# guzba/zippy

Measured on NVIDIA H100. Metric: compress_level1_gzip_input_throughput, higher is better.
Workload: dtype u8

## Files before the change

zippy_b200/csrc/zb_deflate.cu:

```cuda
#include "zb_device.cuh"
#include "zb_kernels.h"
#include "zb_huff_warp.cuh"

#define LZ_THREADS (ZB_WARPS_PER_CHUNK * 32)
#define LZ_HASH_BITS 11
#define LZ_TABLE_ENTRIES (1 << LZ_HASH_BITS)
#define LZ_PRESEED 2048
#ifndef ZB_LZ1_RESOLVE_WINNER
#define ZB_LZ1_RESOLVE_WINNER 0
#endif
#define LZ_LANE_CAP 32

#define LZ_PIECE_BYTES ZB_REC_PIECE_BYTES
#define LZ_PHASES (ZB_SUB_BYTES / LZ_PIECE_BYTES)
#define LZ_PHASE_BYTES (ZB_CHUNK_BYTES / LZ_PHASES)
#define LZ_PHASE_HIST 1024
#define LZ_BATCH_LPW 2
#define LZ_BATCH_WINDOWS (32 / LZ_BATCH_LPW)
static_assert(LZ_PIECE_BYTES * ZB_WARPS_PER_CHUNK == LZ_PHASE_BYTES, "one piece per warp and phase");
static_assert(LZ_PIECE_BYTES / ZB_WINDOW % LZ_BATCH_WINDOWS == 0, "a batch of windows never straddles two pieces");

#define LZ_SM_DATA 0
#define LZ_SM_DATA_BYTES (LZ_PHASE_BYTES + LZ_PHASE_HIST + 64 + 384)
#define LZ_SM_TABLE (LZ_SM_DATA + LZ_SM_DATA_BYTES)
#define LZ_SM_TABLE_BYTES (ZB_WARPS_PER_CHUNK * LZ_TABLE_ENTRIES * 2)
#define LZ_SM_HIST (LZ_SM_TABLE + LZ_SM_TABLE_BYTES)
#define LZ_SM_HIST_BYTES (ZB_WARPS_PER_CHUNK * ZB_HIST_WORDS * 4)
#define LZ_SM_RING (LZ_SM_HIST + LZ_SM_HIST_BYTES)
#define LZ_SM_RING_BYTES (ZB_WARPS_PER_CHUNK * LZ_BATCH_WINDOWS * ZB_MATCH_SLOTS * 4)
#define LZ_SM_LMUL (LZ_SM_RING + LZ_SM_RING_BYTES)
#define LZ_LMUL_PIECE 33
#define LZ_LMUL_PQ 49
#define LZ_SM_LMUL_BYTES (56 * 4)
#define LZ_SM_PART (LZ_SM_LMUL + LZ_SM_LMUL_BYTES)
#define LZ_SM_PART_BYTES (ZB_WARPS_PER_CHUNK * 24)
#define LZ_SM_BAR (LZ_SM_PART + LZ_SM_PART_BYTES)
#define LZ_SM_TOTAL (LZ_SM_BAR + 16)
static_assert(LZ_TABLE_ENTRIES * 2 >= 4096, "a warp's table region must hold the CRC step table");
static_assert(3 * (LZ_SM_TOTAL + 1024) <= 233472, "three CTAs per SM");
static_assert(LZ_SM_PART % 8 == 0 && LZ_SM_TABLE % 16 == 0, "alignment");

__device__ __forceinline__ uint32_t lz_hash(uint32_t v) { return (v * 0x9E3779B1u) >> (32 - LZ_HASH_BITS); }
__device__ __forceinline__ uint32_t shl_clamp(uint32_t x, uint32_t n) {
  uint32_t r;
  asm("shl.b32 %0, %1, %2;" : "=r"(r) : "r"(x), "r"(n));
  return r;
}
__device__ __forceinline__ uint32_t low_mask(uint32_t n) { return shl_clamp(1u, n) - 1u; }

__device__ __forceinline__ uint32_t lz_final_rec(uint32_t mlen, uint32_t dist, int &lc, int &dc) {
  uint32_t le, de;
  lc = (int)zb_len_code_bf(mlen, le);
  dc = (int)zb_dist_code_bf(dist, de);
  return (uint32_t)lc | (le << 5) | ((uint32_t)dc << 10) | (de << 15);
}


__device__ __forceinline__ void lz_select(const uint8_t *data, uint32_t off0, uint32_t wb, uint32_t b1, uint32_t cur,
                                          uint32_t nvalid, uint32_t &m, uint32_t dist, uint32_t *ring_slot,
                                          uint32_t &sel, uint32_t &ism, uint32_t &endw) {
  const int lane = zb_lane();
  const uint32_t mm = __ballot_sync(ZB_FULL, m != 0);
  endw = 0;
  ism = 0;
  if (mm) {
    const uint32_t lbit = 1u << lane;
    const uint32_t endp = (uint32_t)lane + m;
    const uint32_t rest = shl_clamp(1u, endp) ? (mm >> endp) : 0u;
    uint32_t nc = rest ? endp + (uint32_t)(__ffs((int)rest) - 1) : 32u;
    uint32_t vis = 1u << (cur + (uint32_t)(__ffs((int)(mm >> cur)) - 1));
#pragma unroll
    for (int r = 0; r < 3; r++) {
      vis |= __reduce_or_sync(ZB_FULL, (vis & lbit) ? shl_clamp(1u, nc) : 0u);
      const uint32_t t = __shfl_sync(ZB_FULL, nc, (int)(nc & 31u));
      nc = nc < 32u ? t : 32u;
    }
    ism = vis;
    const int lastm = 31 - __clz((int)ism);
    const uint32_t cov = (ism & lbit) ? (low_mask(endp) & ~low_mask((uint32_t)lane)) : 0u;
    const uint32_t covered = __reduce_or_sync(ZB_FULL, cov);
    uint32_t mlast = __shfl_sync(ZB_FULL, m, lastm);
    if (mlast >= LZ_LANE_CAP) {
      const uint32_t md = __shfl_sync(ZB_FULL, dist, lastm);
      const uint32_t pos = wb + (uint32_t)lastm;
      const uint32_t off = off0 + pos + LZ_LANE_CAP + 8u * (uint32_t)lane;
      uint32_t x0 = zb_ld32_unaligned(data, off) ^ zb_ld32_unaligned(data, off - md);
      uint32_t x1 = zb_ld32_unaligned(data, off + 4) ^ zb_ld32_unaligned(data, off + 4 - md);
      uint32_t nm = x0 ? ((uint32_t)(__ffs((int)x0) - 1) >> 3) : 4u + (x1 ? ((uint32_t)(__ffs((int)x1) - 1) >> 3) : 4u);
      uint32_t stop = __ballot_sync(ZB_FULL, nm < 8u);
      if (stop) {
        int first = __ffs((int)stop) - 1;
        mlast = LZ_LANE_CAP + 8u * (uint32_t)first + __shfl_sync(ZB_FULL, nm, first);
      } else {
        mlast = LZ_LANE_CAP + 256u;
      }
      mlast = min(mlast, min((uint32_t)ZB_MAX_MATCH, b1 - pos));
      if (lane == lastm) m = mlast;
    }
    sel = ism | (~covered & ~low_mask(cur) & low_mask(nvalid));
    endw = (uint32_t)lastm + mlast;
    if (ism & lbit) {
      uint32_t rank = (uint32_t)__popc(ism & (lbit - 1u));
      ring_slot[rank] = (m - 3u) | ((dist - 1u) << 9);
    }
  } else {
    sel = low_mask(nvalid) & ~low_mask(cur);
  }
}

template <int LPW, bool LITS>
__device__ __forceinline__ void lz_batch_pass(const uint8_t *wdata, bool active, uint32_t ksel, uint32_t kism,
                                              const uint32_t *ring_win, uint32_t *whist, uint2 *gmask_w,
                                              uint32_t *grecs_piece, uint32_t &rec_base) {
  constexpr int NW = 32 / LPW;
  const uint32_t part = (uint32_t)zb_lane() / NW, wi = (uint32_t)zb_lane() % NW;
  if (active && part == 0) *gmask_w = make_uint2(ksel, kism);
  const uint32_t im = active ? kism : 0u;
  const uint32_t pm = (0xffffffffu >> (32 - 32 / LPW)) << (part * (32 / LPW));
  uint32_t s = (LITS && active) ? (ksel & ~kism & pm) : 0u;
  while (s) {
    const uint32_t bit = (uint32_t)(__ffs((int)s) - 1);
    s &= s - 1;
    const uint32_t sy = wdata[bit];
    atomicAdd(&whist[sy >> 1], 1u << ((sy & 1u) * 16u));
  }
  const uint32_t nmatch = (uint32_t)__popc(im);
  uint32_t incl = nmatch;
#pragma unroll
  for (int o = 1; o < NW; o <<= 1) {
    const uint32_t t = __shfl_up_sync(ZB_FULL, incl, o, NW);
    if (wi >= (uint32_t)o) incl += t;
  }
  uint32_t *grecs_w = grecs_piece + rec_base + incl - nmatch;
  rec_base += __shfl_sync(ZB_FULL, incl, NW - 1);
  for (uint32_t k = part; k < nmatch; k += LPW) {
    const uint32_t raw = ring_win[k];
    int lc, dc;
    const uint32_t fin = lz_final_rec((raw & 511u) + 3u, (raw >> 9) + 1u, lc, dc);
    grecs_w[k] = fin;
    const uint32_t s1 = 257u + (uint32_t)lc, s2 = (uint32_t)ZB_NUM_LITLEN + (uint32_t)dc;
    atomicAdd(&whist[s1 >> 1], 1u << ((s1 & 1u) * 16u));
    atomicAdd(&whist[s2 >> 1], 1u << ((s2 & 1u) * 16u));
  }
}

#ifndef ZB_LZ1_STAGE_CLOCKS
#define ZB_LZ1_STAGE_CLOCKS 0
#endif
enum { LZS_WAIT, LZS_CHECKSUM, LZS_SEED, LZS_PROBE, LZS_EXTEND, LZS_SELECT, LZS_BATCH, LZS_BARRIER, LZS_N };
#if ZB_LZ1_STAGE_CLOCKS
__device__ unsigned long long zb_lz1_stage_clk[LZS_N];
#define LZ_CLK_DECL                          \
  unsigned long long clk_acc[LZS_N] = {};    \
  long long clk_t = clock64();
#define LZ_CLK(s)                            \
  if (MODE == 1) {                           \
    const long long clk_n = clock64();       \
    clk_acc[s] += (unsigned long long)(clk_n - clk_t); \
    clk_t = clk_n;                           \
  }
#define LZ_CLK_PUBLISH()                                                                           \
  if (MODE == 1 && lane == 0) {                                                                    \
    _Pragma("unroll") for (int s_ = 0; s_ < LZS_N; s_++) atomicAdd(&zb_lz1_stage_clk[s_], clk_acc[s_]); \
  }
extern "C" int zb200_lz1_stage_clocks(unsigned long long *out) {
  unsigned long long zero[LZS_N] = {};
  if (cudaMemcpyFromSymbol(out, zb_lz1_stage_clk, sizeof(zero)) != cudaSuccess) return -1;
  return cudaMemcpyToSymbol(zb_lz1_stage_clk, zero, sizeof(zero)) == cudaSuccess ? 0 : -1;
}
#else
#define LZ_CLK_DECL
#define LZ_CLK(s)
#define LZ_CLK_PUBLISH()
#endif

template <int MODE, int CK>
__global__ void __launch_bounds__(LZ_THREADS, 3)
    k_lz(const uint8_t *__restrict__ src, const ZbChunkDesc *__restrict__ desc, uint2 *__restrict__ masks,
         uint32_t *__restrict__ recs, uint16_t *__restrict__ hist, ZbChunkCheck *__restrict__ chk,
         const ZbCrcTables *__restrict__ tabs, uint32_t max_dist) {
  extern __shared__ __align__(128) uint8_t smem[];
  uint8_t *data = smem + LZ_SM_DATA;
  uint16_t *table_all = reinterpret_cast<uint16_t *>(smem + LZ_SM_TABLE);
  uint32_t *hist_all = reinterpret_cast<uint32_t *>(smem + LZ_SM_HIST);
  uint32_t *ring_all = reinterpret_cast<uint32_t *>(smem + LZ_SM_RING);
  uint32_t *lane_mul = reinterpret_cast<uint32_t *>(smem + LZ_SM_LMUL);
  uint64_t *part = reinterpret_cast<uint64_t *>(smem + LZ_SM_PART);
  uint64_t *bar = reinterpret_cast<uint64_t *>(smem + LZ_SM_BAR);

  const uint32_t chunk = blockIdx.x;
  const ZbChunkDesc d = desc[chunk];
  const uint32_t len = d.len;
  const int tid = (int)threadIdx.x, lane = tid & 31;
  const int warp = (int)__reduce_max_sync(ZB_FULL, (uint32_t)tid >> 5);

  if (tid == 0) {
    zb_mbar_init(bar, 1);
    zb_fence_mbar_init();
  }
  __syncthreads();
  const uint32_t mis = (uint32_t)((uintptr_t)(src + d.src_off) & 15u);

  uint16_t *table = table_all + warp * LZ_TABLE_ENTRIES;
  uint32_t *ring = ring_all + warp * LZ_BATCH_WINDOWS * ZB_MATCH_SLOTS;
  uint2 *gmask = masks + (size_t)chunk * ZB_WINDOWS_PER_CHUNK;
  uint32_t acc_crc = 0;
  uint64_t acc_a = 0, acc_b = 0;
  LZ_CLK_DECL

  for (uint32_t ph = 0; ph < LZ_PHASES; ph++) {
    const uint32_t pbase = ph * LZ_PHASE_BYTES;
    if (ph && pbase >= len) break;
    const uint32_t sbase = ph ? pbase - LZ_PHASE_HIST : 0u;
    if (ph) __syncthreads();
    LZ_CLK(LZS_BARRIER)
    if (tid == 0 && len) {
      zb_fence_proxy_async();
      zb_stage_chunk(data, src + d.src_off + sbase, min(len, pbase + LZ_PHASE_BYTES + 384u) - sbase, bar);
    }
    if (CK & ZB_CK_CRC) {
      uint32_t *crc_tab = reinterpret_cast<uint32_t *>(table);
      for (int i = lane; i < 1024; i += 32) crc_tab[i] = (&tabs->mul1024[0][0])[i];
    }
    if (ph == 0) {
      for (int i = tid; i < ZB_WARPS_PER_CHUNK * ZB_HIST_WORDS; i += LZ_THREADS) hist_all[i] = 0;
      if (tid < 33) lane_mul[tid] = tabs->lane_mul[tid];
      if (tid >= 64 && tid < 80) lane_mul[LZ_LMUL_PIECE + tid - 64] = tabs->piece_mul[tid - 64];
      if (tid >= 96 && tid < 100) lane_mul[LZ_LMUL_PQ + tid - 96] = tabs->pq_mul[tid - 96];
      __syncthreads();
    } else {
      __syncwarp();
    }
    if (len) zb_mbar_wait(bar, ph & 1u);
    LZ_CLK(LZS_WAIT)

    const uint32_t b0 = pbase + (uint32_t)warp * LZ_PIECE_BYTES;
    if (b0 >= len) continue;
    const uint32_t b1 = min(b0 + LZ_PIECE_BYTES, len);
    const uint32_t doff = mis - sbase;
    uint32_t *whist = hist_all + (b0 / ZB_SUB_BYTES) * ZB_HIST_WORDS;

    if (CK) {
      ZbCheck c = zb_warp_checksums<LZ_PIECE_BYTES, LZ_LMUL_PQ, CK>(data, doff + b0, b1 - b0,
                                                                    reinterpret_cast<const uint32_t *>(table), lane_mul);
      const uint32_t after = len - b1;
      if (after) {
        if (CK & ZB_CK_CRC) {
          const uint32_t shift = ((after & (LZ_PIECE_BYTES - 1)) == 0) ? lane_mul[LZ_LMUL_PIECE + after / LZ_PIECE_BYTES]
                                                                       : zb_xpow8_t(tabs->pow2, after);
          c.crc_raw = zb_gf2_mul(c.crc_raw, shift);
        }
        if (CK & ZB_CK_ADLER) c.b_sum += (uint64_t)after * c.a_sum;
      }
      acc_crc ^= c.crc_raw;
      acc_a += c.a_sum;
      acc_b += c.b_sum;
      __syncwarp();
    }
    LZ_CLK(LZS_CHECKSUM)

    if (MODE == 1) {
      uint4 ff = make_uint4(~0u, ~0u, ~0u, ~0u);
      uint4 *t4 = reinterpret_cast<uint4 *>(table);
      for (int i = lane; i < LZ_TABLE_ENTRIES * 2 / 16; i += 32) t4[i] = ff;
      __syncwarp();
      for (uint32_t s = b0 - min((uint32_t)LZ_PRESEED, b0 - sbase); s < b0; s += 32) {
        const uint32_t p = s + (uint32_t)lane;
        const bool can = p + 4 <= len;
        const uint32_t h = lz_hash(zb_ld32_unaligned(data, doff + p));
        if (can) table[h] = (uint16_t)p;
#if ZB_LZ1_RESOLVE_WINNER
        __syncwarp();
        for (;;) {
          const bool lost = can && table[h] < (uint16_t)p;
          if (!__any_sync(ZB_FULL, lost)) break;
          if (lost) table[h] = (uint16_t)p;
          __syncwarp();
        }
#endif
      }
      __syncwarp();
    }
    LZ_CLK(LZS_SEED)
    uint32_t entry = b0;
    uint32_t ksel = 0, kism = 0;
    uint32_t *grecs = recs + (size_t)chunk * ZB_RECS_PER_CHUNK + (b0 >> 2);
    uint32_t rec_base = 0;
    const uint32_t bl = (uint32_t)lane & (LZ_BATCH_WINDOWS - 1u);
    for (uint32_t wb = b0; wb < b1; wb += 32) {
      const uint32_t win = wb >> 5, slot = win & (LZ_BATCH_WINDOWS - 1u);
      uint32_t sel = 0, ism = 0;
      if (entry < wb + 32) {
        const uint32_t p = wb + (uint32_t)lane;
        const uint32_t nvalid = min(32u, b1 - wb);
        const uint32_t cur = entry - wb;
        uint32_t m = 0, c = 0, lit = 0;
        if (MODE == 2) {
          const uint32_t x = doff + p;
          lit = data[x];
          const uint32_t eq0 = __ballot_sync(ZB_FULL, p != 0u && lit == data[x - 1u]);
          const uint32_t eq1 = __ballot_sync(ZB_FULL, data[x + 32u] == data[x + 31u]);
          const uint32_t ahead = __funnelshift_r(eq0, eq1, (uint32_t)lane);
          const uint32_t run = ahead == ~0u ? (uint32_t)LZ_LANE_CAP : (uint32_t)(__ffs((int)~ahead) - 1);
          const uint32_t limit = p < b1 ? b1 - p : 0u;
          const uint32_t r = run < (uint32_t)LZ_LANE_CAP ? min(run, limit) : run;
          if (p >= entry && r >= 3u && limit >= 3u) m = r;
          c = p - 1u;
        }
        if (MODE == 1) {
          const uint32_t *wp = reinterpret_cast<const uint32_t *>(data) + ((doff + p) >> 2);
          const uint32_t sp = ((doff + p) & 3u) * 8u;
          const uint32_t p0 = wp[0], p1 = wp[1];
          const uint32_t v = __funnelshift_r(p0, p1, sp);
          lit = v & 255u;
          const bool can = (p + 4 <= len);
          const uint32_t h = lz_hash(v);
          c = table[h];
          __syncwarp();
          if (can) table[h] = (uint16_t)p;
#if ZB_LZ1_RESOLVE_WINNER
          __syncwarp();
          for (;;) {
            const bool lost = can && table[h] < (uint16_t)p;
            if (!__any_sync(ZB_FULL, lost)) break;
            if (lost) table[h] = (uint16_t)p;
            __syncwarp();
          }
#endif
          LZ_CLK(LZS_PROBE)
          const uint32_t limit = p < b1 ? min((uint32_t)ZB_MAX_MATCH, b1 - p) : 0u;
          if (can && c < p && p - c <= max_dist && p >= entry && limit >= ZB_MIN_MATCH) {
            const uint32_t *wc = reinterpret_cast<const uint32_t *>(data) + ((doff + c) >> 2);
            const uint32_t sc = ((doff + c) & 3u) * 8u;
            uint32_t hp = p1, hc = wc[1];
            uint32_t np = wp[2], nq = wc[2], np2 = wp[3], nq2 = wc[3];
            if (__funnelshift_r(wc[0], hc, sc) == v) {
              m = 4;
#pragma unroll 1
              for (int k = 2;; k += 2) {
                const uint32_t x = __funnelshift_r(hp, np, sp) ^ __funnelshift_r(hc, nq, sc);
                const uint32_t x2 = __funnelshift_r(np, np2, sp) ^ __funnelshift_r(nq, nq2, sc);
                if (x) {
                  m += (uint32_t)(__ffs((int)x) - 1) >> 3;
                  break;
                }
                if (k == LZ_LANE_CAP / 4) {
                  m += 4;
                  break;
                }
                if (x2) {
                  m += 4u + ((uint32_t)(__ffs((int)x2) - 1) >> 3);
                  break;
                }
                m += 8;
                hp = np2;
                hc = nq2;
                np = wp[k + 2];
                nq = wc[k + 2];
                np2 = wp[k + 3];
                nq2 = wc[k + 3];
              }
              if (m < LZ_LANE_CAP) m = min(m, limit);
            }
          }
          LZ_CLK(LZS_EXTEND)
        }
        uint32_t endw;
        lz_select(data, doff, wb, b1, cur, nvalid, m, p - c, ring + slot * ZB_MATCH_SLOTS, sel, ism, endw);
        entry = wb + max(endw, nvalid);
        if (MODE != 0 && ((sel & ~ism) >> lane & 1u)) atomicAdd(&whist[lit >> 1], 1u << ((lit & 1u) * 16u));
        LZ_CLK(LZS_SELECT)
      }
      if (bl == slot) {
        ksel = sel;
        kism = ism;
      }
      if (slot == LZ_BATCH_WINDOWS - 1u || wb + 32 >= b1) {
        __syncwarp();
        const uint32_t bwin = win - slot + bl;
        lz_batch_pass<LZ_BATCH_LPW, MODE == 0>(data + (uint32_t)(doff + (bwin << 5)), bl <= slot, ksel, kism, ring + bl * ZB_MATCH_SLOTS,
                                    whist, gmask + bwin, grecs, rec_base);
        ksel = kism = 0;
        __syncwarp();
      }
      LZ_CLK(LZS_BATCH)
    }
  }
  if (lane == 0) {
    part[warp * 3 + 0] = acc_crc;
    part[warp * 3 + 1] = acc_a;
    part[warp * 3 + 2] = acc_b;
  }
  __syncthreads();
  {
    uint32_t *gh = reinterpret_cast<uint32_t *>(hist + (size_t)chunk * ZB_WARPS_PER_CHUNK * ZB_HIST_SYMS);
    for (int i = tid; i < ZB_WARPS_PER_CHUNK * ZB_HIST_WORDS; i += LZ_THREADS) gh[i] = hist_all[i];
  }
  LZ_CLK(LZS_BARRIER)
  LZ_CLK_PUBLISH()
  if (tid == 0) {
    uint32_t raw = 0;
    uint64_t a = 0, b = 0;
    for (int w = 0; w < ZB_WARPS_PER_CHUNK; w++) {
      raw ^= (uint32_t)part[w * 3 + 0];
      a += part[w * 3 + 1];
      b += part[w * 3 + 2];
    }
    ZbChunkCheck cc;
    cc.crc_raw = raw;
    cc.adler = (CK & ZB_CK_ADLER) ? zb_adler_from_sums(a % ZB_ADLER_MOD, b % ZB_ADLER_MOD, len) : 0u;
    chk[chunk] = cc;
  }
}

#define LZ2_HIST 32768
#define LZ2_SEG_BYTES ZB_SUB_BYTES
#define LZ2_SEGS ((ZB_CHUNK_BYTES + LZ2_HIST) / LZ2_SEG_BYTES)
#define LZ2_BUCKET_BITS 11
#define LZ2_BUCKETS (1 << LZ2_BUCKET_BITS)
#define LZ2_TABLES_PER_CTA (ZB_WARPS_PER_CHUNK + LZ2_SEGS)
#define LZ2_RING_WINDOWS 8
#define LZ2_SM_DATA_BYTES (ZB_CHUNK_BYTES + LZ2_HIST + 64 + 384)
#define LZ2_SM_HIST (LZ2_SM_DATA_BYTES)
#define LZ2_SM_RING (LZ2_SM_HIST + LZ_SM_HIST_BYTES)
#define LZ2_SM_RING_BYTES (ZB_WARPS_PER_CHUNK * LZ2_RING_WINDOWS * ZB_MATCH_SLOTS * 4)
#define LZ2_SM_CRC (LZ2_SM_RING + LZ2_SM_RING_BYTES)
#define LZ2_SM_LMUL (LZ2_SM_CRC + 4096)
#define LZ2_SM_PART (LZ2_SM_LMUL + LZ_SM_LMUL_BYTES)
#define LZ2_SM_LIST (LZ2_SM_PART + LZ_SM_PART_BYTES)
#define LZ2_SM_BAR (LZ2_SM_LIST + 8 * LZ_THREADS * 2)
#define LZ2_SM_TOTAL (LZ2_SM_BAR + 16)
static_assert(2 * (LZ2_SM_TOTAL + 1024) <= 233472, "two CTAs per SM");

#ifndef LZ2_CTAS_PER_SM
#define LZ2_CTAS_PER_SM 1
#endif
#ifndef LZ2_STATIC_BITS
#define LZ2_STATIC_BITS 13
#endif
__device__ __forceinline__ uint32_t lz2_hash_mul(uint32_t v) { return v * 0x9E3779B1u; }
__device__ __forceinline__ uint32_t lz2_hash(uint32_t v) { return lz2_hash_mul(v) >> (32 - LZ2_BUCKET_BITS); }

__device__ __forceinline__ uint2 lz2_push(uint2 b, uint32_t e) {
  uint2 r;
  r.y = __funnelshift_l(b.x, b.y, 16);
  r.x = (b.x << 16) | (e & 0xffffu);
  return r;
}

__device__ __forceinline__ void lz2_clear_table(uint2 *tab, int bytes = LZ2_BUCKETS * 8) {
  const uint4 ff = make_uint4(~0u, ~0u, ~0u, ~0u);
  uint4 *t4 = reinterpret_cast<uint4 *>(tab);
  for (int i = zb_lane(); i < bytes / 16; i += 32) __stcg(&t4[i], ff);
}

__device__ __forceinline__ uint2 lz2_probe_insert(uint2 *tab, uint32_t h, bool can, uint32_t qwin, uint32_t &grp) {
  const int lane = zb_lane();
  grp = __match_any_sync(ZB_FULL, can ? h : (0x80000000u | (uint32_t)lane));
  uint2 old = make_uint2(~0u, ~0u);
  if (can) old = __ldcg(&tab[h]);
  __syncwarp();
  if (can && lane == 31 - __clz((int)grp)) {
    uint2 nb = old;
    for (uint32_t g = grp; g; g &= g - 1) nb = lz2_push(nb, qwin + (uint32_t)(__ffs((int)g) - 1));
    __stcg(&tab[h], nb);
  }
  __syncwarp();
  return old;
}

struct Lz2Pos {
  const uint32_t *data32;
  uint32_t poff;
  uint32_t q;
  uint32_t v;
  uint32_t lim;
  uint32_t limit, stop;
};

#define LZ2_LIST 8
__device__ __forceinline__ void lz2_verify(const Lz2Pos &P, uint32_t e, bool search, uint16_t *dl, uint32_t &n) {
  const uint32_t d = (P.q - e) & 0xffffu;
  if (!search || (d - 1u) >= P.lim) return;
  const uint32_t co = P.poff - d;
  const uint32_t *wc = P.data32 + (co >> 2);
  if (__funnelshift_r(wc[0], wc[1], (co & 3u) * 8u) != P.v) return;
  if (n < LZ2_LIST) dl[n * (uint32_t)LZ_THREADS] = (uint16_t)d;
  n += n < LZ2_LIST ? 1u : 0u;
}
__device__ __forceinline__ void lz2_extend(const Lz2Pos &P, const uint8_t *data, uint32_t d, uint32_t good, uint32_t &m,
                                           uint32_t &dist, int &budget) {
  const uint32_t co = P.poff - d;
  budget--;
  if (m >= 4 && data[co + m] != data[P.poff + m]) {
    if (m >= good && budget > 1) budget = 1;
    return;
  }
  const uint32_t *wc = P.data32 + (co >> 2);
  const uint32_t sc = (co & 3u) * 8u;
  const uint32_t *wp = P.data32 + (P.poff >> 2);
  const uint32_t sp = (P.poff & 3u) * 8u;
  uint32_t hp = wp[1], hc = wc[1];
  uint32_t mc = 4;
#pragma unroll 1
  for (int j = 2; j <= LZ_LANE_CAP / 4; j++) {
    const uint32_t np = wp[j], nq = wc[j];
    const uint32_t x = __funnelshift_r(hp, np, sp) ^ __funnelshift_r(hc, nq, sc);
    if (x) {
      mc += (uint32_t)(__ffs((int)x) - 1) >> 3;
      break;
    }
    mc += 4;
    hp = np;
    hc = nq;
  }
  mc = min(mc, P.limit);
  if (mc > m) {
    m = mc;
    dist = d;
  }
  if (m >= good && budget > 1) budget = 1;
}

__device__ __forceinline__ void stage_dict_chunk(uint8_t *data, const uint8_t *chunk, uint32_t len, uint32_t hb,
                                                 const uint8_t *wend, uint64_t *bar) {
  const uint32_t cmis = (uint32_t)((uintptr_t)chunk & 15u);
  const uint32_t mis = (cmis - hb) & 15u, a0 = hb + mis - cmis;
  const uint32_t cbytes = (cmis + len + 15u) & ~15u;
  zb_mbar_expect_tx(bar, a0 + cbytes);
  for (uint32_t done = 0; done < a0;) {
    const uint32_t n = min(a0 - done, 32768u);
    zb_tma_load_1d(data + done, wend - hb - mis + done, n, bar);
    done += n;
  }
  for (uint32_t done = 0; done < cbytes;) {
    const uint32_t n = min(cbytes - done, 32768u);
    zb_tma_load_1d(data + a0 + done, chunk - cmis + done, n, bar);
    done += n;
  }
}
__device__ __forceinline__ void fix_dict_head(uint8_t *data, const uint8_t *chunk, uint32_t hb, const uint8_t *wend) {
  const uint32_t cmis = (uint32_t)((uintptr_t)chunk & 15u);
  const uint32_t mis = (cmis - hb) & 15u;
  const uint32_t q = hb - min(hb, cmis) + threadIdx.x;
  if (q < hb) {
    data[mis + q] = wend[(int)q - (int)hb];
    zb_fence_proxy_async();
  }
}

template <bool DICT, int MINM = ZB_MIN_MATCH>
__global__ void __launch_bounds__(LZ_THREADS, 2)
    k_lz2(const uint8_t *__restrict__ src, const ZbChunkDesc *__restrict__ desc, uint2 *__restrict__ masks,
          uint32_t *__restrict__ recs, uint16_t *__restrict__ hist, ZbChunkCheck *__restrict__ chk,
          const ZbCrcTables *__restrict__ tabs, uint2 *__restrict__ tables, uint32_t n_chunks, ZbLz2Params prm,
          const ZbMemberDict *__restrict__ mdict) {
  extern __shared__ __align__(128) uint8_t smem[];
  uint8_t *data = smem;
  uint32_t *hist_all = reinterpret_cast<uint32_t *>(smem + LZ2_SM_HIST);
  uint32_t *ring_all = reinterpret_cast<uint32_t *>(smem + LZ2_SM_RING);
  uint32_t *crc_tab = reinterpret_cast<uint32_t *>(smem + LZ2_SM_CRC);
  uint32_t *lane_mul = reinterpret_cast<uint32_t *>(smem + LZ2_SM_LMUL);
  uint64_t *part = reinterpret_cast<uint64_t *>(smem + LZ2_SM_PART);
  uint64_t *bar = reinterpret_cast<uint64_t *>(smem + LZ2_SM_BAR);
  const int tid = (int)threadIdx.x, lane = tid & 31, warp = tid >> 5;
  uint16_t *dlist = reinterpret_cast<uint16_t *>(smem + LZ2_SM_LIST) + tid;
  uint32_t *whist = hist_all + warp * ZB_HIST_WORDS;
  uint32_t *ring = ring_all + warp * LZ2_RING_WINDOWS * ZB_MATCH_SLOTS;
  uint2 *cta_tabs = tables + (size_t)blockIdx.x * LZ2_TABLES_PER_CTA * LZ2_BUCKETS;
  uint2 *own = cta_tabs + (size_t)warp * LZ2_BUCKETS;
  uint2 *stat = cta_tabs + (size_t)ZB_WARPS_PER_CHUNK * LZ2_BUCKETS;

  if (tid == 0) {
    zb_mbar_init(bar, 1);
    zb_fence_mbar_init();
  }
  for (int i = tid; i < 1024; i += LZ_THREADS) crc_tab[i] = (&tabs->mul1024[0][0])[i];
  if (tid < 33) lane_mul[tid] = tabs->lane_mul[tid];
  if (tid >= 64 && tid < 72) lane_mul[33 + tid - 64] = tabs->sub_mul[tid - 64];
  if (tid >= 96 && tid < 100) lane_mul[41 + tid - 96] = tabs->quart_mul[tid - 96];
  __syncthreads();

  uint32_t phase = 0;
  for (uint32_t chunk = blockIdx.x; chunk < n_chunks; chunk += gridDim.x) {
    const ZbChunkDesc d = desc[chunk];
    const uint32_t len = d.len, hb = d.pad;
    const uint32_t hg = (0u - hb) & (LZ2_SEG_BYTES - 1u);
    const uint8_t *rsrc = src + d.src_off - hb;
    const uint32_t mis = (uint32_t)((uintptr_t)rsrc & 15u);
    const uint32_t off0 = mis + hb;
    const uint32_t rlen = hb + len;
    const uint8_t *wend = DICT && (d.flags & ZB_CHUNK_DICT) ? mdict[d.member].wend : nullptr;
    if (DICT && wend) {
      if (tid == 0) stage_dict_chunk(data, src + d.src_off, len, hb, wend, bar);
    } else if (tid == 0 && rlen) {
      zb_stage_chunk(data, rsrc, rlen, bar);
    }
    for (int i = tid; i < ZB_WARPS_PER_CHUNK * ZB_HIST_WORDS; i += LZ_THREADS) hist_all[i] = 0;
    lz2_clear_table(own);
    __syncthreads();
    if (rlen) {
      zb_mbar_wait(bar, phase);
      phase ^= 1u;
    }
    if (DICT && wend) {
      fix_dict_head(data, src + d.src_off, hb, wend);
      __syncthreads();
    }

    const uint32_t b0 = (uint32_t)warp * ZB_SUB_BYTES;
    const uint32_t b1 = min(b0 + ZB_SUB_BYTES, len);
    {
      ZbCheck c;
      c.crc_raw = 0;
      c.a_sum = c.b_sum = 0;
      uint32_t n = b0 < len ? b1 - b0 : 0;
      if (n) {
        c = zb_warp_checksums(data, off0 + b0, n, crc_tab, lane_mul);
        const uint32_t after = len - b1;
        if (after) {
          const uint32_t shift = ((after & (ZB_SUB_BYTES - 1)) == 0) ? lane_mul[33 + after / ZB_SUB_BYTES] : zb_xpow8_t(tabs->pow2, after);
          c.crc_raw = zb_gf2_mul(c.crc_raw, shift);
          c.b_sum += (uint64_t)after * c.a_sum;
        }
      }
      if (lane == 0) {
        part[warp * 3 + 0] = c.crc_raw;
        part[warp * 3 + 1] = c.a_sum;
        part[warp * 3 + 2] = c.b_sum;
      }
      __syncwarp();
    }

    {
      const uint32_t nseg = (hg + rlen + LZ2_SEG_BYTES - 1) / LZ2_SEG_BYTES;
      const uint32_t seg0 = (hg + hb) / LZ2_SEG_BYTES, sg0 = seg0 > prm.hist_segs ? seg0 - prm.hist_segs : 0u;
      for (uint32_t sg = sg0 + (uint32_t)warp; sg + 1 < nseg; sg += ZB_WARPS_PER_CHUNK) {
        uint2 *tab = stat + (size_t)sg * LZ2_BUCKETS;
        lz2_clear_table(tab, (1 << LZ2_STATIC_BITS) * 2);
        __syncwarp();
        uint16_t *tab16 = reinterpret_cast<uint16_t *>(tab);
        const uint32_t q0 = sg ? sg * LZ2_SEG_BYTES - hg : 0u, q1 = (sg + 1) * LZ2_SEG_BYTES - hg;
        for (uint32_t s = q0; s < q1; s += 32) {
          const uint32_t q = s + (uint32_t)lane;
          const uint32_t v = zb_ld32_unaligned(data, mis + q);
          const uint32_t hs = lz2_hash_mul(v) >> (32 - LZ2_STATIC_BITS);
          const bool can = q + 4 <= rlen && q < q1;
          const uint32_t grp = __match_any_sync(ZB_FULL, can ? hs : (0x80000000u | (uint32_t)lane));
          if (can && lane == 31 - __clz((int)grp)) __stcg(&tab16[hs], (uint16_t)q);
        }
        __syncwarp();
      }
    }
    __syncthreads();

    if (b0 < len) {
      const uint32_t myseg = (hg + hb + b0) / LZ2_SEG_BYTES;
      uint32_t entry = b0;
      uint32_t ksel = 0, kism = 0;
      uint2 *gmask = masks + (size_t)chunk * ZB_WINDOWS_PER_CHUNK;
      uint32_t *grecs = recs + (size_t)chunk * ZB_RECS_PER_CHUNK;
      uint32_t rec_base = 0;
      for (uint32_t wb = b0; wb < b1; wb += 32) {
        const uint32_t win = wb >> 5, slot = win & (LZ2_RING_WINDOWS - 1u);
        if ((wb & (ZB_REC_PIECE_BYTES - 1u)) == 0u) rec_base = 0;
        const uint32_t p = wb + (uint32_t)lane;
        const uint32_t q = hb + p;
        const uint32_t v = zb_ld32_unaligned(data, off0 + p);
        const bool can = (p + 4 <= len);
        const uint32_t h = lz2_hash(v);
        const uint32_t limit = p < b1 ? min((uint32_t)ZB_MAX_MATCH, b1 - p) : 0u;
        const bool search = entry < wb + 32 && can && p >= entry && limit >= ZB_MIN_MATCH;
        const uint32_t hs = lz2_hash_mul(v) >> (32 - LZ2_STATIC_BITS);
        uint32_t hcand[4];
#pragma unroll
        for (int j = 0; j < 4; j++) {
          hcand[j] = 0xffffu;
          if (search && myseg > (uint32_t)j && prm.hist_segs > (uint32_t)j)
            hcand[j] = __ldcg(reinterpret_cast<const uint16_t *>(stat + (size_t)(myseg - 1u - (uint32_t)j) * LZ2_BUCKETS) + hs);
        }
        uint32_t grp;
        const uint2 bucket = lz2_probe_insert(own, h, can, q - (uint32_t)lane, grp);
        uint32_t sel = 0, ism = 0;
        if (entry < wb + 32) {
          const uint32_t nvalid = min(32u, b1 - wb);
          const uint32_t cur = entry - wb;
          uint32_t m = 0, dist = 1;
          int budget = search ? (int)prm.maxcand : 0;
// ... 685 lines not shown
```

Measured before the change: 80.62.

## Software-pipeline LZ level-1 hash probe of next window with current select

Splits the level-1 match finder into probe, check and extend stages and, when no lane hit the 32-byte lane cap, issues the hash-table probe and first match check for the next 32-byte window before running warp-wide selection on the current one. This overlaps shared/global load latency of the next window with the ballot and shuffle work of selection. A branchless first-check path replaces the data-dependent branch, and an uncapped lz_select variant drops the long-match extension step. The cost is more live registers and extra speculative loads and table updates for positions that may later be skipped.

```diff
diff --git a/zippy_b200/csrc/zb_deflate.cu b/zippy_b200/csrc/zb_deflate.cu
--- a/zippy_b200/csrc/zb_deflate.cu
+++ b/zippy_b200/csrc/zb_deflate.cu
@@ -56,6 +56,7 @@
 }
 
 
+template <bool CAPPED = true>
 __device__ __forceinline__ void lz_select(const uint8_t *data, uint32_t off0, uint32_t wb, uint32_t b1, uint32_t cur,
                                           uint32_t nvalid, uint32_t &m, uint32_t dist, uint32_t *ring_slot,
                                           uint32_t &sel, uint32_t &ism, uint32_t &endw) {
@@ -63,12 +64,12 @@
   const uint32_t mm = __ballot_sync(ZB_FULL, m != 0);
   endw = 0;
   ism = 0;
-  if (mm) {
+  if (!CAPPED || mm) {
     const uint32_t lbit = 1u << lane;
     const uint32_t endp = (uint32_t)lane + m;
     const uint32_t rest = shl_clamp(1u, endp) ? (mm >> endp) : 0u;
     uint32_t nc = rest ? endp + (uint32_t)(__ffs((int)rest) - 1) : 32u;
-    uint32_t vis = 1u << (cur + (uint32_t)(__ffs((int)(mm >> cur)) - 1));
+    uint32_t vis = CAPPED ? 1u << (cur + (uint32_t)(__ffs((int)(mm >> cur)) - 1)) : mm & (0u - mm);
 #pragma unroll
     for (int r = 0; r < 3; r++) {
       vis |= __reduce_or_sync(ZB_FULL, (vis & lbit) ? shl_clamp(1u, nc) : 0u);
@@ -80,7 +81,7 @@
     const uint32_t cov = (ism & lbit) ? (low_mask(endp) & ~low_mask((uint32_t)lane)) : 0u;
     const uint32_t covered = __reduce_or_sync(ZB_FULL, cov);
     uint32_t mlast = __shfl_sync(ZB_FULL, m, lastm);
-    if (mlast >= LZ_LANE_CAP) {
+    if (CAPPED && mlast >= LZ_LANE_CAP) {
       const uint32_t md = __shfl_sync(ZB_FULL, dist, lastm);
       const uint32_t pos = wb + (uint32_t)lastm;
       const uint32_t off = off0 + pos + LZ_LANE_CAP + 8u * (uint32_t)lane;
@@ -98,14 +99,98 @@
       if (lane == lastm) m = mlast;
     }
     sel = ism | (~covered & ~low_mask(cur) & low_mask(nvalid));
-    endw = (uint32_t)lastm + mlast;
-    if (ism & lbit) {
-      uint32_t rank = (uint32_t)__popc(ism & (lbit - 1u));
-      ring_slot[rank] = (m - 3u) | ((dist - 1u) << 9);
-    }
+    endw = (CAPPED || ism) ? (uint32_t)lastm + mlast : 0u;
+    const uint32_t rank = (uint32_t)__popc(ism & (lbit - 1u));
+    const uint32_t rec = (m - 3u) | ((dist - 1u) << 9);
+    if (ism & lbit) ring_slot[rank] = rec;
   } else {
     sel = low_mask(nvalid) & ~low_mask(cur);
   }
+}
+
+struct Lz1Lane {
+  uint32_t c, lit, m;
+  uint32_t limit;
+  uint32_t ip, ic;
+  uint32_t sp, sc;
+  uint32_t hp, hc;
+  bool more;
+};
+
+__device__ __forceinline__ void lz1_probe(const uint8_t *data, uint16_t *table, uint32_t doff, uint32_t p,
+                                          uint32_t len, Lz1Lane &L, uint32_t &v, bool &can) {
+  const uint32_t *w = reinterpret_cast<const uint32_t *>(data);
+  L.ip = (doff + p) >> 2;
+  L.sp = ((doff + p) & 3u) * 8u;
+  L.hp = w[L.ip + 1];
+  v = __funnelshift_r(w[L.ip], L.hp, L.sp);
+  L.lit = v & 255u;
+  can = p + 4 <= len;
+  const uint32_t h = lz_hash(v);
+  L.c = table[h];
+  __syncwarp();
+  if (can) table[h] = (uint16_t)p;
+#if ZB_LZ1_RESOLVE_WINNER
+  __syncwarp();
+  for (;;) {
+    const bool lost = can && table[h] < (uint16_t)p;
+    if (!__any_sync(ZB_FULL, lost)) break;
+    if (lost) table[h] = (uint16_t)p;
+    __syncwarp();
+  }
+#endif
+}
+
+__device__ __forceinline__ void lz1_check(const uint8_t *data, uint32_t doff, uint32_t p, uint32_t b1,
+                                          uint32_t max_dist, uint32_t v, bool can, Lz1Lane &L) {
+  const uint32_t *w = reinterpret_cast<const uint32_t *>(data);
+  L.limit = p < b1 ? min((uint32_t)ZB_MAX_MATCH, b1 - p) : 0u;
+  const bool ok = can && L.c < p && p - L.c <= max_dist && L.limit >= ZB_MIN_MATCH;
+  const uint32_t q = ok ? L.c : p;
+  L.ic = (doff + q) >> 2;
+  L.sc = ((doff + q) & 3u) * 8u;
+  const uint32_t c0 = w[L.ic], hc = w[L.ic + 1];
+  const uint32_t np = w[L.ip + 2], nq = w[L.ic + 2], np2 = w[L.ip + 3], nq2 = w[L.ic + 3];
+  const uint32_t x = __funnelshift_r(L.hp, np, L.sp) ^ __funnelshift_r(hc, nq, L.sc);
+  const uint32_t x2 = __funnelshift_r(np, np2, L.sp) ^ __funnelshift_r(nq, nq2, L.sc);
+  const bool hit = ok && __funnelshift_r(c0, hc, L.sc) == v;
+  const uint32_t tx = __clz((int)__brev(x)), tx2 = __clz((int)__brev(x2));
+  const uint32_t eq = (tx + (x ? 0u : tx2)) >> 3;
+  L.m = hit ? 4u + eq : 0u;
+  L.more = hit && eq == 8u;
+  L.hp = np2;
+  L.hc = nq2;
+}
+
+__device__ __forceinline__ void lz1_extend(const uint8_t *data, bool before_entry, Lz1Lane &L) {
+  const uint32_t *w = reinterpret_cast<const uint32_t *>(data);
+  if (before_entry) {
+    L.m = 0;
+  } else if (L.more) {
+    uint32_t hp = L.hp, hc = L.hc;
+#pragma unroll 1
+    for (uint32_t k = 4;; k += 2) {
+      const uint32_t np = w[L.ip + k], nq = w[L.ic + k], np2 = w[L.ip + k + 1], nq2 = w[L.ic + k + 1];
+      const uint32_t x = __funnelshift_r(hp, np, L.sp) ^ __funnelshift_r(hc, nq, L.sc);
+      const uint32_t x2 = __funnelshift_r(np, np2, L.sp) ^ __funnelshift_r(nq, nq2, L.sc);
+      if (x) {
+        L.m += (uint32_t)(__ffs((int)x) - 1) >> 3;
+        break;
+      }
+      if (k == LZ_LANE_CAP / 4) {
+        L.m += 4;
+        break;
+      }
+      if (x2) {
+        L.m += 4u + ((uint32_t)(__ffs((int)x2) - 1) >> 3);
+        break;
+      }
+      L.m += 8;
+      hp = np2;
+      hc = nq2;
+    }
+  }
+  if (L.m < LZ_LANE_CAP) L.m = min(L.m, L.limit);
 }
 
 template <int LPW, bool LITS>
@@ -287,90 +372,8 @@
     uint32_t *grecs = recs + (size_t)chunk * ZB_RECS_PER_CHUNK + (b0 >> 2);
     uint32_t rec_base = 0;
     const uint32_t bl = (uint32_t)lane & (LZ_BATCH_WINDOWS - 1u);
-    for (uint32_t wb = b0; wb < b1; wb += 32) {
+    auto window_done = [&](uint32_t wb, uint32_t sel, uint32_t ism) {
       const uint32_t win = wb >> 5, slot = win & (LZ_BATCH_WINDOWS - 1u);
-      uint32_t sel = 0, ism = 0;
-      if (entry < wb + 32) {
-        const uint32_t p = wb + (uint32_t)lane;
-        const uint32_t nvalid = min(32u, b1 - wb);
-        const uint32_t cur = entry - wb;
-        uint32_t m = 0, c = 0, lit = 0;
-        if (MODE == 2) {
-          const uint32_t x = doff + p;
-          lit = data[x];
-          const uint32_t eq0 = __ballot_sync(ZB_FULL, p != 0u && lit == data[x - 1u]);
-          const uint32_t eq1 = __ballot_sync(ZB_FULL, data[x + 32u] == data[x + 31u]);
-          const uint32_t ahead = __funnelshift_r(eq0, eq1, (uint32_t)lane);
-          const uint32_t run = ahead == ~0u ? (uint32_t)LZ_LANE_CAP : (uint32_t)(__ffs((int)~ahead) - 1);
-          const uint32_t limit = p < b1 ? b1 - p : 0u;
-          const uint32_t r = run < (uint32_t)LZ_LANE_CAP ? min(run, limit) : run;
-          if (p >= entry && r >= 3u && limit >= 3u) m = r;
-          c = p - 1u;
-        }
-        if (MODE == 1) {
-          const uint32_t *wp = reinterpret_cast<const uint32_t *>(data) + ((doff + p) >> 2);
-          const uint32_t sp = ((doff + p) & 3u) * 8u;
-          const uint32_t p0 = wp[0], p1 = wp[1];
-          const uint32_t v = __funnelshift_r(p0, p1, sp);
-          lit = v & 255u;
-          const bool can = (p + 4 <= len);
-          const uint32_t h = lz_hash(v);
-          c = table[h];
-          __syncwarp();
-          if (can) table[h] = (uint16_t)p;
-#if ZB_LZ1_RESOLVE_WINNER
-          __syncwarp();
-          for (;;) {
-            const bool lost = can && table[h] < (uint16_t)p;
-            if (!__any_sync(ZB_FULL, lost)) break;
-            if (lost) table[h] = (uint16_t)p;
-            __syncwarp();
-          }
-#endif
-          LZ_CLK(LZS_PROBE)
-          const uint32_t limit = p < b1 ? min((uint32_t)ZB_MAX_MATCH, b1 - p) : 0u;
-          if (can && c < p && p - c <= max_dist && p >= entry && limit >= ZB_MIN_MATCH) {
-            const uint32_t *wc = reinterpret_cast<const uint32_t *>(data) + ((doff + c) >> 2);
-            const uint32_t sc = ((doff + c) & 3u) * 8u;
-            uint32_t hp = p1, hc = wc[1];
-            uint32_t np = wp[2], nq = wc[2], np2 = wp[3], nq2 = wc[3];
-            if (__funnelshift_r(wc[0], hc, sc) == v) {
-              m = 4;
-#pragma unroll 1
-              for (int k = 2;; k += 2) {
-                const uint32_t x = __funnelshift_r(hp, np, sp) ^ __funnelshift_r(hc, nq, sc);
-                const uint32_t x2 = __funnelshift_r(np, np2, sp) ^ __funnelshift_r(nq, nq2, sc);
-                if (x) {
-                  m += (uint32_t)(__ffs((int)x) - 1) >> 3;
-                  break;
-                }
-                if (k == LZ_LANE_CAP / 4) {
-                  m += 4;
-                  break;
-                }
-                if (x2) {
-                  m += 4u + ((uint32_t)(__ffs((int)x2) - 1) >> 3);
-                  break;
-                }
-                m += 8;
-                hp = np2;
-                hc = nq2;
-                np = wp[k + 2];
-                nq = wc[k + 2];
-                np2 = wp[k + 3];
-                nq2 = wc[k + 3];
-              }
-              if (m < LZ_LANE_CAP) m = min(m, limit);
-            }
-          }
-          LZ_CLK(LZS_EXTEND)
-        }
-        uint32_t endw;
-        lz_select(data, doff, wb, b1, cur, nvalid, m, p - c, ring + slot * ZB_MATCH_SLOTS, sel, ism, endw);
-        entry = wb + max(endw, nvalid);
-        if (MODE != 0 && ((sel & ~ism) >> lane & 1u)) atomicAdd(&whist[lit >> 1], 1u << ((lit & 1u) * 16u));
-        LZ_CLK(LZS_SELECT)
-      }
       if (bl == slot) {
         ksel = sel;
         kism = ism;
@@ -378,12 +381,84 @@
       if (slot == LZ_BATCH_WINDOWS - 1u || wb + 32 >= b1) {
         __syncwarp();
         const uint32_t bwin = win - slot + bl;
-        lz_batch_pass<LZ_BATCH_LPW, MODE == 0>(data + (uint32_t)(doff + (bwin << 5)), bl <= slot, ksel, kism, ring + bl * ZB_MATCH_SLOTS,
-                                    whist, gmask + bwin, grecs, rec_base);
+        lz_batch_pass<LZ_BATCH_LPW, MODE == 0>(data + (uint32_t)(doff + (bwin << 5)), bl <= slot, ksel, kism,
+                                               ring + bl * ZB_MATCH_SLOTS, whist, gmask + bwin, grecs, rec_base);
         ksel = kism = 0;
         __syncwarp();
       }
       LZ_CLK(LZS_BATCH)
+    };
+    if (MODE == 1) {
+      Lz1Lane L;
+      bool ahead = false;
+      for (uint32_t wb = b0; wb < b1; wb += 32) {
+        uint32_t *ring_win = ring + ((wb >> 5) & (LZ_BATCH_WINDOWS - 1u)) * ZB_MATCH_SLOTS;
+        uint32_t sel = 0, ism = 0;
+        if (entry < wb + 32) {
+          const uint32_t p = wb + (uint32_t)lane;
+          const uint32_t nvalid = min(32u, b1 - wb);
+          const uint32_t cur = entry - wb;
+          uint32_t v, endw;
+          bool can;
+          if (!ahead) {
+            lz1_probe(data, table, doff, p, len, L, v, can);
+            LZ_CLK(LZS_PROBE)
+            lz1_check(data, doff, p, b1, max_dist, v, can, L);
+            lz1_extend(data, p < entry, L);
+            LZ_CLK(LZS_EXTEND)
+          }
+          ahead = wb + 32 < b1 && !__any_sync(ZB_FULL, L.m >= LZ_LANE_CAP);
+          if (ahead) {
+            Lz1Lane N;
+            lz1_probe(data, table, doff, p + 32, len, N, v, can);
+            lz1_check(data, doff, p + 32, b1, max_dist, v, can, N);
+            lz_select<false>(data, doff, wb, b1, cur, nvalid, L.m, p - L.c, ring_win, sel, ism, endw);
+            entry = wb + max(endw, nvalid);
+            uint32_t *hw = &whist[L.lit >> 1];
+            const uint32_t one = 1u << ((L.lit & 1u) * 16u);
+            if ((sel & ~ism) >> lane & 1u) atomicAdd(hw, one);
+            LZ_CLK(LZS_SELECT)
+            lz1_extend(data, p + 32 < entry, N);
+            L = N;
+            LZ_CLK(LZS_EXTEND)
+          } else {
+            lz_select(data, doff, wb, b1, cur, nvalid, L.m, p - L.c, ring_win, sel, ism, endw);
+            entry = wb + max(endw, nvalid);
+            if ((sel & ~ism) >> lane & 1u) atomicAdd(&whist[L.lit >> 1], 1u << ((L.lit & 1u) * 16u));
+            LZ_CLK(LZS_SELECT)
+          }
+        }
+        window_done(wb, sel, ism);
+      }
+    } else {
+      for (uint32_t wb = b0; wb < b1; wb += 32) {
+        uint32_t sel = 0, ism = 0;
+        if (entry < wb + 32) {
+          const uint32_t p = wb + (uint32_t)lane;
+          const uint32_t nvalid = min(32u, b1 - wb);
+          const uint32_t cur = entry - wb;
+          uint32_t m = 0, c = 0, lit = 0;
+          if (MODE == 2) {
+            const uint32_t x = doff + p;
+            lit = data[x];
+            const uint32_t eq0 = __ballot_sync(ZB_FULL, p != 0u && lit == data[x - 1u]);
+            const uint32_t eq1 = __ballot_sync(ZB_FULL, data[x + 32u] == data[x + 31u]);
+            const uint32_t ahead = __funnelshift_r(eq0, eq1, (uint32_t)lane);
+            const uint32_t run = ahead == ~0u ? (uint32_t)LZ_LANE_CAP : (uint32_t)(__ffs((int)~ahead) - 1);
+            const uint32_t limit = p < b1 ? b1 - p : 0u;
+            const uint32_t r = run < (uint32_t)LZ_LANE_CAP ? min(run, limit) : run;
+            if (p >= entry && r >= 3u && limit >= 3u) m = r;
+            c = p - 1u;
+          }
+          uint32_t endw;
+          lz_select(data, doff, wb, b1, cur, nvalid, m, p - c, ring + ((wb >> 5) & (LZ_BATCH_WINDOWS - 1u)) * ZB_MATCH_SLOTS,
+                    sel, ism, endw);
+          entry = wb + max(endw, nvalid);
+          if (MODE == 2 && ((sel & ~ism) >> lane & 1u)) atomicAdd(&whist[lit >> 1], 1u << ((lit & 1u) * 16u));
+          LZ_CLK(LZS_SELECT)
+        }
+        window_done(wb, sel, ism);
+      }
     }
   }
   if (lane == 0) {
```

New measurement: 83.37, median of 6. +3.4%, better.
